# Wuziyi616/SlotDiffusion

Measured on AMD Instinct MI355X. Metric: train-step images/sec, 128x128 7-slot (DPM-Solver denoise-steps/sec in `denoise`), higher is better.
Workload: dtype bf16; 1 GPU; BASELINE configs[1]: img_based SlotDiffusion, CLEVRTex 128x128, 7 slots: train step = slot encoder + frozen VQ-VAE encode + q-sample + UNet eps + MSE, backward, clip, Adam (dropout 0.1); batch_per_gpu=64, hip_graph=True, parallelism=dp1

## Files before the change

include/sdmi.h:

```cpp
#ifndef SDMI_H_
#define SDMI_H_

#ifdef __cplusplus
extern "C" {
#endif

#define SDMI_VERSION 100

enum { SDMI_F32 = 0, SDMI_BF16 = 1, SDMI_FP8 = 2  };
enum { SDMI_ACT_NONE = 0, SDMI_ACT_RELU = 1, SDMI_ACT_SILU = 2, SDMI_ACT_GELU = 3 };
enum { SDMI_OK = 0, SDMI_EINVAL = -1, SDMI_ELAUNCH = -2, SDMI_EUNSUPPORTED = -3 };

int sdmi_version(void);
const char* sdmi_last_error(void);

typedef struct {
  const void* a;
  const void* w;
  void* out;
  const float* bias;
  const float* rowvec;
  const void* residual;
  float* workspace;
  int dtype, out_dtype;
// ... 21 lines not shown
  void* out2;
  int ldc2;
  int defer_epilogue;
  float* gn_part;
  int gn_groups;
  const float* alpha_dev;
  int parity4;
} SdmiGemmArgs;
int sdmi_igemm(const SdmiGemmArgs* a, void* stream);
int sdmi_igemm_split_plan(const SdmiGemmArgs* a, void* stream);
int sdmi_splitk_finish(const SdmiGemmArgs* a, void* stream);
enum {
  SDMI_ROUTE_NONE = 0,
  SDMI_ROUTE_CFG = 1,
  SDMI_ROUTE_DMA = 2,
  SDMI_ROUTE_SYM = 3,
  SDMI_ROUTE_HALO = 4,
  SDMI_ROUTE_C64 = 5
};
int sdmi_igemm_last_route(void);

typedef struct {
  const void* a;
  const void* dy;
  float* dw;
  float* dbias;
  float* workspace;
  int dtype;
  int M, N, K, lda, ldy;
  int B, H, W, Cin, Ho, Wo, KH, KW, stride, pad_t, pad_l, ups;
  int splits;
  int accumulate;
  int defer_fold;
} SdmiWgradArgs;
int sdmi_wgrad(const SdmiWgradArgs* a, void* stream);
enum {
  SDMI_WGRAD_KERNEL_IGEMM = 0,
  SDMI_WGRAD_KERNEL_C64 = 1,
  SDMI_WGRAD_KERNEL_HALO = 2,
  SDMI_WGRAD_KERNEL_F32_T128 = 3,
  SDMI_WGRAD_KERNEL_F32_T64 = 4
};
int sdmi_wgrad_kernel(const SdmiWgradArgs* a, void* stream);

typedef struct { const void* problems; int n; } SdmiWgradGroupArgs;
int sdmi_wgrad_group(const SdmiWgradGroupArgs* a, void* stream);
int sdmi_wgrad_fold_group(const SdmiWgradGroupArgs* a, void* stream);

typedef struct {
  const void* dgrad; const void* wgrad; const void* fold;
  int dgrad_cap, wgrad_tile;
} SdmiBwdPairArgs;
int sdmi_bwd_pair(const SdmiBwdPairArgs* a, void* stream);

typedef struct {
  const void* x;
  void* y;
  const float* gamma;
  const float* beta;
  float* stats;
  float* partial;
  int dtype;
  int B, HW, C, groups;
  float eps;
  int act;
  int nsplit;
  const void* residual;
  float drop_p;
  long long drop_seed;
  const long long* drop_seed_dev;
  void* y8;
  float y8_scale;
  const void* x2;
  int C1;
  const float* part;
  int part_splits;
  float part_alpha;
  const float* part_bias;
  const float* part_rowvec;
  int part_ldrv;
  const void* part_residual;
  void* raw_out;
} SdmiGroupNormArgs;
int sdmi_groupnorm_stats(const SdmiGroupNormArgs* a, void* stream);
int sdmi_groupnorm_apply(const SdmiGroupNormArgs* a, void* stream);
int sdmi_groupnorm(const SdmiGroupNormArgs* a, void* stream);

typedef struct {
  const void* x;
  const void* dy;
  void* dx;
  const float* gamma;
  const float* beta;
  const float* stats;
  float* dgamma;
  float* dbeta;
  float* partial;
  int dtype;
  int B, HW, C, groups;
  int act;
  int nsplit;
  const void* residual;
  void* dresidual;
  int accumulate;
  const void* dextra0;
  const void* dextra1;
  float drop_p;
  long long drop_seed;
  const long long* drop_seed_dev;
  float* dxsum;
  int ld_dxsum;
  int defer_colsum;
} SdmiGroupNormBwdArgs;
int sdmi_groupnorm_bwd(const SdmiGroupNormBwdArgs* a, void* stream);
int sdmi_groupnorm_bwd_fused(const SdmiGroupNormBwdArgs* a, void* unused);
int sdmi_groupnorm_bwd_entries(const SdmiGroupNormBwdArgs* a, void* stream);

typedef struct {
  const void* x; void* y; const float* gamma; const float* beta;
  float* stats;
  int dtype; int rows, C, ldx, ldy; float eps;
} SdmiLayerNormArgs;
int sdmi_layernorm(const SdmiLayerNormArgs* a, void* stream);

typedef struct {
  const void* x; const void* dy; void* dx; const float* gamma; const float* stats;
  float* dgamma; float* dbeta;
  float* partial;
  int dtype; int rows, C; int nblk; int accumulate;
  const void* dextra;
  int defer_colsum;
} SdmiLayerNormBwdArgs;
int sdmi_layernorm_bwd(const SdmiLayerNormBwdArgs* a, void* stream);

typedef struct { const float* partial; float* out0; float* out1; int nblk, C; } SdmiColsumItem;
typedef struct { const void* items; int n; } SdmiColsumGroupArgs;
int sdmi_colsum_group(const SdmiColsumGroupArgs* a, void* stream);


typedef struct {
  const void* q; const void* k; const void* v; void* out; float* lse;
  int dtype; int B, heads, Sq, Skv; int ldq, ldk, ldv, ldo; float scale;
  int head_dim;
} SdmiAttnArgs;
int sdmi_attention(const SdmiAttnArgs* a, void* stream);

typedef struct {
  const void* q; const void* k; const void* v; const void* out; const void* dout; const float* lse;
  void* dq; void* dk; void* dv;
  int dtype; int B, heads, Sq, Skv; int ldq, ldk, ldv, ldo; float scale;
  int head_dim;
} SdmiAttnBwdArgs;
int sdmi_attention_bwd(const SdmiAttnBwdArgs* a, void* stream);

typedef struct { void* x; int dtype; int rows, cols, ld; float scale; } SdmiSoftmaxArgs;
int sdmi_softmax_rows(const SdmiSoftmaxArgs* a, void* stream);

typedef struct {
  const void* k; const void* v;
  const float* slots_in;
  float* slots_out;
  float* seg;
  const float *lnq_g, *lnq_b, *wq;
  const float *w_ih, *w_hh, *b_ih, *b_hh;
  const float *lnm_g, *lnm_b, *w1, *b1, *w2, *b2;
  float* trace;
  int dtype; int B, M, N, D, Hid, iters, ldkv; long long slots_bstride; float eps, scale;
} SdmiSlotAttnArgs;
int sdmi_slot_attention(const SdmiSlotAttnArgs* a, void* stream);

typedef struct {
  const float* z; const float* codebook; long long* idx; float* zq;
  int R, dim, ldz, n_codes; float scale;
  const float* z2; float zc0, zc1, zdiv;
} SdmiVqArgs;
int sdmi_vq_nearest(const SdmiVqArgs* a, void* stream);

enum { SDMI_DPM_EPS = 0, SDMI_DPM_X0 = 1, SDMI_DPM_V = 2 };
enum { SDMI_DPM_UPD_NONE = 0, SDMI_DPM_UPD_FIRST = 1, SDMI_DPM_UPD_SINGLE = 2, SDMI_DPM_UPD_MULTI2 = 3,
       SDMI_DPM_UPD_MULTI3 = 4 };
typedef struct {
  const float* x; const float* out; const float* codebook;
  long long* idx; float* m0;
  const float* base; const float* h1; const float* h2; float* y;
  int R, n_codes, target, mode;
  float scale, sigma, alpha;
  float c0, c1, c2, c3, k0, k1, g, k2;
} SdmiDpmStepArgs;
int sdmi_dpm_step(const SdmiDpmStepArgs* a, void* stream);

typedef struct {
  const float* x; const float* out; const float* codebook;
  long long* idx; float* m0;
  int R, n_codes, target;
  float scale, sigma, alpha;
  const float* base; const float* h1; const float* h2; const float* h3;
  float* xc; float* y;
  int corr_order, pred_order;
  float c0, c1, w1, w2, wn;
  float p0, p1, q1, q2;
} SdmiUnipcStepArgs;
int sdmi_unipc_step(const SdmiUnipcStepArgs* a, void* stream);

enum { SDMI_X0_NONE = 0, SDMI_X0_CLAMP = 1, SDMI_X0_DYNAMIC = 2 };
enum { SDMI_PX_MAX_ROWS = 16384 };
typedef struct {
  const float* x; const float* out; float* m0;
  const float* base; const float* h1; const float* h2; float* y;
  int R, rows_per_sample, target, mode, correct, q_k;
  float q_w, max_val, sigma, alpha;
  float c0, c1, c2, c3, k0, k1, g, k2;
} SdmiDpmStepPxArgs;
int sdmi_dpm_step_px(const SdmiDpmStepPxArgs* a, void* stream);

typedef struct {
  const float* x; const float* out; float* m0;
  int R, rows_per_sample, target, correct, q_k;
  float q_w, max_val, sigma, alpha;
  const float* base; const float* h1; const float* h2; const float* h3;
  float* xc; float* y;
  int corr_order, pred_order;
  float c0, c1, w1, w2, wn;
  float p0, p1, q1, q2;
} SdmiUnipcStepPxArgs;
int sdmi_unipc_step_px(const SdmiUnipcStepPxArgs* a, void* stream);

typedef struct {
  float* y; const float* x0; const float* x1; const float* x2; const float* x3;
  float c0, c1, c2, div; long long n;
} SdmiLincombArgs;
int sdmi_lincomb(const SdmiLincombArgs* a, void* stream);
typedef struct {
  float* y; const float* x0; const float* x1; const float* ca; const float* cb; int B; long long per;
} SdmiRowLincombArgs;
int sdmi_row_lincomb(const SdmiRowLincombArgs* a, void* stream);

typedef struct { const float* src; void* dst; int dtype; int B, C, H, W, Cpad; } SdmiNchwToNhwcArgs;
int sdmi_nchw_to_nhwc(const SdmiNchwToNhwcArgs* a, void* stream);
typedef struct { const void* src; float* dst; int dtype; int B, C, H, W, Cpad; } SdmiNhwcToNchwArgs;
int sdmi_nhwc_to_nchw(const SdmiNhwcToNchwArgs* a, void* stream);
typedef struct {
  const void* src; void* dst; int src_dtype, dst_dtype; long long rows; int cols, lds, ldd;
  int zpad;
} SdmiCast2dArgs;
int sdmi_cast2d(const SdmiCast2dArgs* a, void* stream);
typedef struct {
  const void* src; void* dst; int src_dtype; long long rows; int cols, lds, ldd; float scale;
} SdmiQuantFp8Args;
int sdmi_quant_fp8(const SdmiQuantFp8Args* a, void* stream);
typedef struct { const void* src; void* dst; long long n; int block_begin; int pad_; } SdmiFp8Desc;
typedef struct {
  const void* descs; int n_desc; int src_dtype; int total_blocks;
  unsigned* amax_bits;
  float* inv_scale;
} SdmiFp8GroupArgs;
int sdmi_fp8_quant_group(const SdmiFp8GroupArgs* a, void* stream);
typedef struct {
  const void* x; void* tok; void* qkv; void* out;
  const float* gn_gamma; const float* gn_beta;
  const void* wstream_a; const float* vec_a;
  const void* wstream_b; const float* vec_b;
  const void* wstream_img; const float* vec_img;
  int B, S, C, slots, phase;
  float gn_eps, ln_eps, attn_scale;
  int rows;
  float* part; int ff_split;
} SdmiStBlockArgs;
int sdmi_st_block(const SdmiStBlockArgs* a, void* stream);

typedef struct {
  const void* x; void* qkv; void* out;
  const void* wstream_a; const float* vec_a;
  const void* wstream_b; const float* vec_b;
  int B, L, Lp, C, heads, ffn_dim, phase;
  float ln_eps, attn_scale;
} SdmiRolloutLayerArgs;
int sdmi_rollout_layer(const SdmiRolloutLayerArgs* a, void* stream);

enum { SDMI_AGG_SUM = 0, SDMI_AGG_MEAN = 1, SDMI_AGG_MAX = 2 };
typedef struct {
  const void* slots; const void* w1p; const float* b1; const float* w2; const float* b2;
  const float* label;
  float* frame_logits; float* logits; int* t_star; float* loss; float* dlogit;
  int B, T, N, C, F, agg, x_dtype, op_dtype, phase;
  float loss_weight;
} SdmiReadoutFwdArgs;
int sdmi_readout_fwd(const SdmiReadoutFwdArgs* a, void* stream);
typedef struct {
  const void* slots; const void* w1p; const float* b1; const float* w2;
  const int* t_star; const float* dlogit; const float* gscale;
  float* dw1; float* db1; float* dw2; float* db2;
  int B, T, N, C, F, agg, x_dtype, op_dtype, accumulate;
} SdmiReadoutBwdArgs;
int sdmi_readout_bwd(const SdmiReadoutBwdArgs* a, void* stream);

typedef struct {
  const void* x; void* out;
  void* hgn; float* gn_stats;
  void* tok; void* n1; float* st1; void* qkv;
  void* a1; float* lse1;
  void* x1; void* n2; float* st2;
  void* q2; void* a2; float* lse2;
  void* x2; void* n3; float* st3;
  void* h; void* g; void* x3;
  const void* kv2; int ldkv;
  const void* wstream_a; const void* wstream_b;
// ... 223 lines not shown
```

slotdiffusion_amd/csrc/attention_bwd.hip:

```cpp
#include "common.h"

namespace {

template <typename T, int HD>
__device__ __forceinline__ void load_row32(const T* p, float* f) {
  constexpr int VEC = Elem<T>::VEC;
#pragma unroll
  for (int c = 0; c < HD; c += VEC) unpack16<T>(*reinterpret_cast<const uint4*>(p + c), f + c);
}
template <typename T, int HD>
__device__ __forceinline__ void store_row32(T* p, const float* f) {
  constexpr int VEC = Elem<T>::VEC;
#pragma unroll
  for (int c = 0; c < HD; c += VEC) *reinterpret_cast<uint4*>(p + c) = pack16<T>(f + c);
}

template <typename T, int HD>
__global__ __launch_bounds__(256) void attn_bwd_dq_kernel(SdmiAttnBwdArgs p) {
  constexpr int VEC = Elem<T>::VEC;
  extern __shared__ __attribute__((aligned(16))) char smem[];
  float* Ks = reinterpret_cast<float*>(smem);
  float* Vs = Ks + p.Skv * HD;
  const int b = blockIdx.z, h = blockIdx.y, tid = threadIdx.x;
  {
    const int vpr = HD / VEC, total = p.Skv * vpr;
    const T* kb = (const T*)p.k + (long long)b * p.Skv * p.ldk + h * HD;
    const T* vb = (const T*)p.v + (long long)b * p.Skv * p.ldv + h * HD;
    for (int i = tid; i < total; i += blockDim.x) {
      const int row = i / vpr, c = (i % vpr) * VEC;
      float f[VEC];
      unpack16<T>(*reinterpret_cast<const uint4*>(kb + (long long)row * p.ldk + c), f);
#pragma unroll
      for (int j = 0; j < VEC; ++j) Ks[row * HD + c + j] = f[j];
      unpack16<T>(*reinterpret_cast<const uint4*>(vb + (long long)row * p.ldv + c), f);
#pragma unroll
      for (int j = 0; j < VEC; ++j) Vs[row * HD + c + j] = f[j];
    }
  }
  __syncthreads();
  const int qi = blockIdx.x * blockDim.x + tid;
  if (qi >= p.Sq) return;
  float q[HD], dO[HD], o[HD], dq[HD];
  load_row32<T, HD>((const T*)p.q + ((long long)b * p.Sq + qi) * p.ldq + h * HD, q);
  load_row32<T, HD>((const T*)p.dout + ((long long)b * p.Sq + qi) * p.ldo + h * HD, dO);
  load_row32<T, HD>((const T*)p.out + ((long long)b * p.Sq + qi) * p.ldo + h * HD, o);
  float D = 0.f;
#pragma unroll
  for (int d = 0; d < HD; ++d) { D += dO[d] * o[d]; dq[d] = 0.f; q[d] *= p.scale; }
  const float lse = p.lse[((long long)b * p.heads + h) * p.Sq + qi];
  for (int j = 0; j < p.Skv; ++j) {
    float s = 0.f, dp = 0.f;
#pragma unroll
    for (int d = 0; d < HD; ++d) { s += q[d] * Ks[j * HD + d]; dp += dO[d] * Vs[j * HD + d]; }
    const float ds = __expf(s - lse) * (dp - D);
#pragma unroll
    for (int d = 0; d < HD; ++d) dq[d] += ds * Ks[j * HD + d];
  }
#pragma unroll
  for (int d = 0; d < HD; ++d) dq[d] *= p.scale;
  store_row32<T, HD>((T*)p.dq + ((long long)b * p.Sq + qi) * p.ldq + h * HD, dq);
}

template <typename T, int HD>
__global__ __launch_bounds__(256) void attn_bwd_dkv_kernel(SdmiAttnBwdArgs p) {
  constexpr int VEC = Elem<T>::VEC;
  constexpr int QC = 64;
  __shared__ float Qs[QC][HD], Os[QC][HD], Ts[QC][HD], Ls[QC], Ds[QC];
  const int b = blockIdx.z, h = blockIdx.y, tid = threadIdx.x;
  const int kj = blockIdx.x * blockDim.x + tid;
  const bool act = kj < p.Skv;
  float k[HD], v[HD], dk[HD], dv[HD];
  if (act) {
    load_row32<T, HD>((const T*)p.k + ((long long)b * p.Skv + kj) * p.ldk + h * HD, k);
    load_row32<T, HD>((const T*)p.v + ((long long)b * p.Skv + kj) * p.ldv + h * HD, v);
  }
#pragma unroll
  for (int d = 0; d < HD; ++d) { dk[d] = dv[d] = 0.f; if (!act) k[d] = v[d] = 0.f; }
  for (int q0 = 0; q0 < p.Sq; q0 += QC) {
    __syncthreads();
    const int vpr = HD / VEC;
    for (int i = tid; i < QC * vpr; i += blockDim.x) {
      const int r = i / vpr, c = (i % vpr) * VEC, qi = q0 + r;
      float fq[VEC], fo[VEC], fout[VEC];
      if (qi < p.Sq) {
        const long long ro = ((long long)b * p.Sq + qi);
        unpack16<T>(*reinterpret_cast<const uint4*>((const T*)p.q + ro * p.ldq + h * HD + c), fq);
        unpack16<T>(*reinterpret_cast<const uint4*>((const T*)p.dout + ro * p.ldo + h * HD + c), fo);
        unpack16<T>(*reinterpret_cast<const uint4*>((const T*)p.out + ro * p.ldo + h * HD + c), fout);
      } else {
#pragma unroll
        for (int j = 0; j < VEC; ++j) fq[j] = fo[j] = fout[j] = 0.f;
      }
#pragma unroll
      for (int j = 0; j < VEC; ++j) { Qs[r][c + j] = fq[j]; Os[r][c + j] = fo[j]; Ts[r][c + j] = fout[j]; }
    }
    __syncthreads();
    for (int r = tid; r < QC; r += blockDim.x) {
      const int qi = q0 + r;
      float D = 0.f;
#pragma unroll
      for (int d = 0; d < HD; ++d) D += Os[r][d] * Ts[r][d];
      Ds[r] = D;
      Ls[r] = qi < p.Sq ? p.lse[((long long)b * p.heads + h) * p.Sq + qi] : INFINITY;
    }
    __syncthreads();
    const int qn = min(QC, p.Sq - q0);
    for (int r = 0; r < qn; ++r) {
      float s = 0.f, dp = 0.f;
#pragma unroll
      for (int d = 0; d < HD; ++d) { s += Qs[r][d] * k[d]; dp += Os[r][d] * v[d]; }
      const float pij = __expf(s * p.scale - Ls[r]);
      const float ds = pij * (dp - Ds[r]);
#pragma unroll
      for (int d = 0; d < HD; ++d) { dv[d] += pij * Os[r][d]; dk[d] += ds * Qs[r][d]; }
    }
  }
  if (!act) return;
#pragma unroll
  for (int d = 0; d < HD; ++d) dk[d] *= p.scale;
  store_row32<T, HD>((T*)p.dk + ((long long)b * p.Skv + kj) * p.ldk + h * HD, dk);
  store_row32<T, HD>((T*)p.dv + ((long long)b * p.Skv + kj) * p.ldv + h * HD, dv);
}

template <typename T, int HD>
__global__ __launch_bounds__(512) void attn_bwd_dkv_small_kernel(SdmiAttnBwdArgs p) {
  const int b = blockIdx.y, h = blockIdx.x;
  const int j = threadIdx.x / HD, d = threadIdx.x % HD;
  const float kd = Elem<T>::ld((const T*)p.k + ((long long)b * p.Skv + j) * p.ldk + h * HD + d);
  const float vd = Elem<T>::ld((const T*)p.v + ((long long)b * p.Skv + j) * p.ldv + h * HD + d);
  const float* lse = p.lse + ((long long)b * p.heads + h) * p.Sq;
  float dk = 0.f, dv = 0.f;
  for (int i = 0; i < p.Sq; ++i) {
    const long long ro = (long long)b * p.Sq + i;
    const float qd = Elem<T>::ld((const T*)p.q + ro * p.ldq + h * HD + d);
    const float od = Elem<T>::ld((const T*)p.dout + ro * p.ldo + h * HD + d);
    const float outd = Elem<T>::ld((const T*)p.out + ro * p.ldo + h * HD + d);
    float s = qd * kd, dp = od * vd, D = od * outd;
#pragma unroll
    for (int o = 16; o > 0; o >>= 1) {
      s += __shfl_xor(s, o, 64);
      dp += __shfl_xor(dp, o, 64);
      D += __shfl_xor(D, o, 64);
    }
    const float pij = __expf(s * p.scale - lse[i]);
    dv += pij * od;
    dk += pij * (dp - D) * qd;
  }
  Elem<T>::st((T*)p.dk + ((long long)b * p.Skv + j) * p.ldk + h * HD + d, dk * p.scale);
  Elem<T>::st((T*)p.dv + ((long long)b * p.Skv + j) * p.ldv + h * HD + d, dv);
}

template <typename T, int HD>
int launch_attn_bwd(const SdmiAttnBwdArgs& a, hipStream_t st) {
  int threads = ((a.Sq + 63) / 64) * 64;
  if (threads > 256) threads = 256;
  dim3 grid((a.Sq + threads - 1) / threads, a.heads, a.B);
  const int smem = 2 * a.Skv * HD * 4;
  SDMI_OPTIN_LDS((attn_bwd_dq_kernel<T, HD>), (2 * 512 * HD * 4 < 160 * 1024 ? 2 * 512 * HD * 4 : 160 * 1024),
                 "attention_bwd");
  hipLaunchKernelGGL((attn_bwd_dq_kernel<T, HD>), grid, dim3(threads), smem, st, a);
  if (a.Skv <= 16 && HD == 32) {
    hipLaunchKernelGGL((attn_bwd_dkv_small_kernel<T, HD>), dim3(a.heads, a.B), dim3(a.Skv * HD), 0,
                       st, a);
  } else {
    int kt = ((a.Skv + 63) / 64) * 64;
    if (kt > 256) kt = 256;
    dim3 g2((a.Skv + kt - 1) / kt, a.heads, a.B);
    hipLaunchKernelGGL((attn_bwd_dkv_kernel<T, HD>), g2, dim3(kt), 0, st, a);
  }
  return sdmi_check_launch("attention_bwd");
}


typedef short b_s16x4 __attribute__((ext_vector_type(4)));
typedef short b_s16x8 __attribute__((ext_vector_type(8)));
#define ATB_LDS_V4(p) ((__attribute__((address_space(3))) b_s16x4*)(p))
constexpr int P80 = 80, P64 = 64;

__device__ __forceinline__ unsigned bpack2(float lo, float hi) {
  return (unsigned)f32_to_bf16(lo) | ((unsigned)f32_to_bf16(hi) << 16);
}
__device__ __forceinline__ bf16x8 bpack8(const float* v) {
  const u32x4 w = {bpack2(v[0], v[1]), bpack2(v[2], v[3]), bpack2(v[4], v[5]), bpack2(v[6], v[7])};
  return __builtin_bit_cast(bf16x8, w);
}
__device__ __forceinline__ bf16x8 tr_operand(const char* img_lane, int row0) {
  const char* q = img_lane + row0 * P64;
  const b_s16x4 lo = __builtin_amdgcn_ds_read_tr16_b64_v4i16(ATB_LDS_V4(q));
  const b_s16x4 hi = __builtin_amdgcn_ds_read_tr16_b64_v4i16(ATB_LDS_V4(q + 8 * P64));
  const b_s16x8 v = __builtin_shufflevector(lo, hi, 0, 1, 2, 3, 4, 5, 6, 7);
  return __builtin_bit_cast(bf16x8, v);
}
__device__ __forceinline__ float dot8(const u32x4& a, const u32x4& b) {
  float fa[8], fb[8];
  unpack16<bf16_t>(reinterpret_cast<const uint4&>(a), fa);
  unpack16<bf16_t>(reinterpret_cast<const uint4&>(b), fb);
  float s = 0.f;
#pragma unroll
  for (int i = 0; i < 8; ++i) s += fa[i] * fb[i];
  return s;
}
__device__ __forceinline__ void store_col(bf16_t* rp, const f32x16& acc, float sc) {
#pragma unroll
  for (int j = 0; j < 4; ++j) {
    uint2 w;
    w.x = bpack2(acc[4 * j] * sc, acc[4 * j + 1] * sc);
    w.y = bpack2(acc[4 * j + 2] * sc, acc[4 * j + 3] * sc);
    *reinterpret_cast<uint2*>(rp + 8 * j) = w;
  }
}

constexpr int ATB_CHUNK = 512;

__device__ __forceinline__ void attn_bwd_dq_mfma_body(const SdmiAttnBwdArgs& p, char* smem, int bx, int chunk) {
  const int skv_pad = (p.Skv + 31) / 32 * 32;
  const int cap = skv_pad < chunk ? skv_pad : chunk;
  char* K80 = smem;
  char* K64 = K80 + cap * P80;
  char* V80 = K64 + cap * P64;
  const int b = blockIdx.z, h = blockIdx.y;
  const int tid = threadIdx.x, lane = tid & 63, wave = tid >> 6;
  const int q0 = (bx * 4 + wave) * 32;
  const bool active = q0 < p.Sq;
  const int ql = lane & 31, hh = lane >> 5;
  const int qi = q0 + ql, qc = qi < p.Sq ? qi : p.Sq - 1;
  bf16x8 bq[2], bdo[2];
  float D;
  {
    const long long ro = (long long)b * p.Sq + qc;
    const bf16_t* qp = (const bf16_t*)p.q + ro * p.ldq + h * 32 + hh * 8;
    const bf16_t* dp_ = (const bf16_t*)p.dout + ro * p.ldo + h * 32 + hh * 8;
    const bf16_t* op = (const bf16_t*)p.out + ro * p.ldo + h * 32 + hh * 8;
    const u32x4 q0v = *reinterpret_cast<const u32x4*>(qp), q1v = *reinterpret_cast<const u32x4*>(qp + 16);
    const u32x4 d0v = *reinterpret_cast<const u32x4*>(dp_), d1v = *reinterpret_cast<const u32x4*>(dp_ + 16);
    const u32x4 o0v = *reinterpret_cast<const u32x4*>(op), o1v = *reinterpret_cast<const u32x4*>(op + 16);
    bq[0] = __builtin_bit_cast(bf16x8, q0v); bq[1] = __builtin_bit_cast(bf16x8, q1v);
    bdo[0] = __builtin_bit_cast(bf16x8, d0v); bdo[1] = __builtin_bit_cast(bf16x8, d1v);
    D = dot8(d0v, o0v) + dot8(d1v, o1v);
    D += __shfl_xor(D, 32, 64);
  }
  const float lse = p.lse[((long long)b * p.heads + h) * p.Sq + qc];
  f32x16 dq;
#pragma unroll
  for (int r = 0; r < 16; ++r) dq[r] = 0.f;
  const int g = lane >> 4, t = lane & 15;
  const char* kfrag = K80 + ql * P80 + hh * 16;
  const char* vfrag = V80 + ql * P80 + hh * 16;
  const char* ktr = K64 + (4 * hh + (t >> 2)) * P64 + ((g & 1) * 16 + (t & 3) * 4) * 2;
  const bf16_t* kbase = (const bf16_t*)p.k + (long long)b * p.Skv * p.ldk + h * 32;
  const bf16_t* vbase = (const bf16_t*)p.v + (long long)b * p.Skv * p.ldv + h * 32;
  for (int c0 = 0; c0 < skv_pad; c0 += chunk) {
    const int rows = skv_pad - c0 < chunk ? skv_pad - c0 : chunk;
    if (c0) __syncthreads();
    {
      const u32x4 zero4 = {0u, 0u, 0u, 0u};
      for (int i = tid; i < rows * 4; i += 256) {
        const int row = i >> 2, c = i & 3;
        const bool ok = c0 + row < p.Skv;
        const u32x4 kv = ok ? *reinterpret_cast<const u32x4*>(kbase + (long long)(c0 + row) * p.ldk + c * 8) : zero4;
        const u32x4 vv = ok ? *reinterpret_cast<const u32x4*>(vbase + (long long)(c0 + row) * p.ldv + c * 8) : zero4;
        *reinterpret_cast<u32x4*>(K80 + row * P80 + c * 16) = kv;
        *reinterpret_cast<u32x4*>(K64 + row * P64 + c * 16) = kv;
        *reinterpret_cast<u32x4*>(V80 + row * P80 + c * 16) = vv;
      }
    }
    __syncthreads();
    if (!active) continue;
    for (int kb = 0; kb < rows / 32; ++kb) {
      f32x16 s, dp;
#pragma unroll
      for (int r = 0; r < 16; ++r) s[r] = dp[r] = 0.f;
#pragma unroll
      for (int ks = 0; ks < 2; ++ks) {
        const u32x4 ak = *reinterpret_cast<const u32x4*>(kfrag + kb * 32 * P80 + ks * 32);
        const u32x4 av = *reinterpret_cast<const u32x4*>(vfrag + kb * 32 * P80 + ks * 32);
        s = __builtin_amdgcn_mfma_f32_32x32x16_bf16(__builtin_bit_cast(bf16x8, ak), bq[ks], s, 0, 0, 0);
        dp = __builtin_amdgcn_mfma_f32_32x32x16_bf16(__builtin_bit_cast(bf16x8, av), bdo[ks], dp, 0, 0, 0);
      }
      float ds[16];
#pragma unroll
      for (int r = 0; r < 16; ++r) {
        const int key = c0 + kb * 32 + (r & 3) + 8 * (r >> 2) + 4 * hh;
        const float pr = key < p.Skv ? __expf(s[r] * p.scale - lse) : 0.f;
        ds[r] = pr * (dp[r] - D);
      }
#pragma unroll
      for (int mm = 0; mm < 2; ++mm)
        dq = __builtin_amdgcn_mfma_f32_32x32x16_bf16(tr_operand(ktr, kb * 32 + 16 * mm),
                                                     bpack8(ds + 8 * mm), dq, 0, 0, 0);
    }
  }
  if (active && qi < p.Sq)
    store_col((bf16_t*)p.dq + ((long long)b * p.Sq + qi) * p.ldq + h * 32 + 4 * hh, dq, p.scale);
}

__device__ __forceinline__ void attn_bwd_dkv_mfma_body(const SdmiAttnBwdArgs& p, char* smem, int bx, int chunk) {
  const int sq_pad = (p.Sq + 31) / 32 * 32;
  const int cap = sq_pad < chunk ? sq_pad : chunk;
  char* Q80 = smem;
  char* Q64 = Q80 + cap * P80;
  char* O80 = Q64 + cap * P64;
  char* O64 = O80 + cap * P80;
  float* lse_s = reinterpret_cast<float*>(O64 + cap * P64);
  float* D_s = lse_s + cap;
  const int b = blockIdx.z, h = blockIdx.y;
  const int tid = threadIdx.x, lane = tid & 63, wave = tid >> 6;
  const int k0 = (bx * 4 + wave) * 32;
  const bool active = k0 < p.Skv;
  const int kl = lane & 31, hh = lane >> 5;
  const int kj = k0 + kl, kc = kj < p.Skv ? kj : p.Skv - 1;
  bf16x8 bk[2], bv[2];
  {
    const bf16_t* kp = (const bf16_t*)p.k + ((long long)b * p.Skv + kc) * p.ldk + h * 32 + hh * 8;
    const bf16_t* vp = (const bf16_t*)p.v + ((long long)b * p.Skv + kc) * p.ldv + h * 32 + hh * 8;
    bk[0] = __builtin_bit_cast(bf16x8, *reinterpret_cast<const u32x4*>(kp));
    bk[1] = __builtin_bit_cast(bf16x8, *reinterpret_cast<const u32x4*>(kp + 16));
    bv[0] = __builtin_bit_cast(bf16x8, *reinterpret_cast<const u32x4*>(vp));
    bv[1] = __builtin_bit_cast(bf16x8, *reinterpret_cast<const u32x4*>(vp + 16));
  }
  f32x16 dk, dv;
#pragma unroll
  for (int r = 0; r < 16; ++r) dk[r] = dv[r] = 0.f;
  const int g = lane >> 4, t = lane & 15;
  const char* qfrag = Q80 + kl * P80 + hh * 16;
  const char* ofrag = O80 + kl * P80 + hh * 16;
  const int troff = (4 * hh + (t >> 2)) * P64 + ((g & 1) * 16 + (t & 3) * 4) * 2;
  const char* qtr = Q64 + troff;
  const char* otr = O64 + troff;
  const bf16_t* qb_ = (const bf16_t*)p.q + (long long)b * p.Sq * p.ldq + h * 32;
  const bf16_t* db = (const bf16_t*)p.dout + (long long)b * p.Sq * p.ldo + h * 32;
  const bf16_t* ob = (const bf16_t*)p.out + (long long)b * p.Sq * p.ldo + h * 32;
  for (int c0 = 0; c0 < sq_pad; c0 += chunk) {
    const int rows = sq_pad - c0 < chunk ? sq_pad - c0 : chunk;
    if (c0) __syncthreads();
    {
      const u32x4 zero4 = {0u, 0u, 0u, 0u};
      for (int i = tid; i < rows * 4; i += 256) {
        const int row = i >> 2, c = i & 3;
        const bool ok = c0 + row < p.Sq;
        const u32x4 qv = ok ? *reinterpret_cast<const u32x4*>(qb_ + (long long)(c0 + row) * p.ldq + c * 8) : zero4;
        const u32x4 dv4 = ok ? *reinterpret_cast<const u32x4*>(db + (long long)(c0 + row) * p.ldo + c * 8) : zero4;
        *reinterpret_cast<u32x4*>(Q80 + row * P80 + c * 16) = qv;
        *reinterpret_cast<u32x4*>(Q64 + row * P64 + c * 16) = qv;
        *reinterpret_cast<u32x4*>(O80 + row * P80 + c * 16) = dv4;
        *reinterpret_cast<u32x4*>(O64 + row * P64 + c * 16) = dv4;
      }
      for (int r = tid; r < rows; r += 256) {
        const int qi = c0 + r;
        float d = 0.f, l = INFINITY;
        if (qi < p.Sq) {
#pragma unroll
          for (int c = 0; c < 4; ++c)
            d += dot8(*reinterpret_cast<const u32x4*>(db + (long long)qi * p.ldo + c * 8),
                      *reinterpret_cast<const u32x4*>(ob + (long long)qi * p.ldo + c * 8));
          l = p.lse[((long long)b * p.heads + h) * p.Sq + qi];
        }
        D_s[r] = d;
        lse_s[r] = l;
      }
    }
    __syncthreads();
    if (!active) continue;
    for (int qb = 0; qb < rows / 32; ++qb) {
      f32x16 s, dp;
#pragma unroll
      for (int r = 0; r < 16; ++r) s[r] = dp[r] = 0.f;
#pragma unroll
      for (int ks = 0; ks < 2; ++ks) {
        const u32x4 aq = *reinterpret_cast<const u32x4*>(qfrag + qb * 32 * P80 + ks * 32);
        const u32x4 ao = *reinterpret_cast<const u32x4*>(ofrag + qb * 32 * P80 + ks * 32);
        s = __builtin_amdgcn_mfma_f32_32x32x16_bf16(__builtin_bit_cast(bf16x8, aq), bk[ks], s, 0, 0, 0);
        dp = __builtin_amdgcn_mfma_f32_32x32x16_bf16(__builtin_bit_cast(bf16x8, ao), bv[ks], dp, 0, 0, 0);
      }
      float pr[16], ds[16];
#pragma unroll
      for (int j = 0; j < 4; ++j) {
        const f32x4 l4 = *reinterpret_cast<const f32x4*>(lse_s + qb * 32 + 8 * j + 4 * hh);
        const f32x4 d4 = *reinterpret_cast<const f32x4*>(D_s + qb * 32 + 8 * j + 4 * hh);
#pragma unroll
        for (int i = 0; i < 4; ++i) {
          const int r = 4 * j + i;
          pr[r] = __expf(s[r] * p.scale - l4[i]);
          ds[r] = pr[r] * (dp[r] - d4[i]);
        }
      }
#pragma unroll
      for (int mm = 0; mm < 2; ++mm) {
        dv = __builtin_amdgcn_mfma_f32_32x32x16_bf16(tr_operand(otr, qb * 32 + 16 * mm),
                                                     bpack8(pr + 8 * mm), dv, 0, 0, 0);
        dk = __builtin_amdgcn_mfma_f32_32x32x16_bf16(tr_operand(qtr, qb * 32 + 16 * mm),
                                                     bpack8(ds + 8 * mm), dk, 0, 0, 0);
      }
    }
  }
  if (active && kj < p.Skv) {
    store_col((bf16_t*)p.dk + ((long long)b * p.Skv + kj) * p.ldk + h * 32 + 4 * hh, dk, p.scale);
    store_col((bf16_t*)p.dv + ((long long)b * p.Skv + kj) * p.ldv + h * 32 + 4 * hh, dv, 1.f);
  }
}

__global__ __launch_bounds__(256) void attn_bwd_mfma_kernel(SdmiAttnBwdArgs p, int nqx, int chunk_k, int chunk_q) {
  extern __shared__ __attribute__((aligned(16))) char smem[];
  if ((int)blockIdx.x < nqx) attn_bwd_dq_mfma_body(p, smem, blockIdx.x, chunk_k);
  else attn_bwd_dkv_mfma_body(p, smem, (int)blockIdx.x - nqx, chunk_q);
}

int launch_attn_bwd_mfma(const SdmiAttnBwdArgs& a, hipStream_t st) {
  SDMI_OPTIN_LDS(attn_bwd_mfma_kernel, 160 * 1024, "attention_bwd (mfma)");
  int skv_pad = (a.Skv + 31) / 32 * 32, sq_pad = (a.Sq + 31) / 32 * 32;
  if (skv_pad > ATB_CHUNK) skv_pad = ATB_CHUNK;
  const int qmax = a.Skv <= 32 ? 128 : ATB_CHUNK;
  if (sq_pad > qmax) sq_pad = qmax;
  const int smem_q = skv_pad * (2 * P80 + P64), smem_k = sq_pad * (2 * P80 + 2 * P64 + 8);
  const int nqx = (a.Sq + 127) / 128, nkx = (a.Skv + 127) / 128;
  hipLaunchKernelGGL(attn_bwd_mfma_kernel, dim3(nqx + nkx, a.heads, a.B), dim3(256),
                     smem_q > smem_k ? smem_q : smem_k, st, a, nqx, skv_pad, sq_pad);
  return sdmi_check_launch("attention_bwd (mfma)");
}

}

extern "C" int sdmi_attention_bwd(const SdmiAttnBwdArgs* a, void* stream) {
  SDMI_REQUIRE(a && a->q && a->k && a->v && a->out && a->dout && a->lse && a->dq && a->dk && a->dv,
               "null pointer");
  const int vec = a->dtype == SDMI_BF16 ? 8 : 4;
  SDMI_REQUIRE(a->ldq % vec == 0 && a->ldk % vec == 0 && a->ldv % vec == 0 && a->ldo % vec == 0,
               "row pitches must keep 16-byte alignment");
  const int hd = a->head_dim > 0 ? a->head_dim : 32;
  SDMI_REQUIRE(hd == 32 || hd == 48, "head_dim must be 32 or 48");
  hipStream_t st = (hipStream_t)stream;
  if (a->dtype == SDMI_BF16 && hd == 32) {
    SDMI_REQUIRE(a->Skv >= 1, "Skv must be positive");
    return launch_attn_bwd_mfma(*a, st);
  }
  SDMI_REQUIRE(a->Skv >= 1 && a->Skv <= 400, "Skv must be in [1, 400] (fp32 / head_dim 48: K/V staged whole in LDS)");
  if (a->dtype == SDMI_BF16)
    return hd == 32 ? launch_attn_bwd<bf16_t, 32>(*a, st) : launch_attn_bwd<bf16_t, 48>(*a, st);
  return hd == 32 ? launch_attn_bwd<float, 32>(*a, st) : launch_attn_bwd<float, 48>(*a, st);
}
```

Baseline: 2375 images/s.

## Add single-block-per-head fused MFMA attention backward for short sequences

Adds a new attention-backward kernel that handles one (batch, head) per workgroup when Sq and Skv are at most 256. It stages K/V and Q/dO once in LDS, and each wave does either a dQ row tile or a dK/dV column tile, so the old chunked loop with separate dq and dkv block groups is avoided. It also pairs heads to remap block indices, skips key masking on full tiles, and uses a paired bf16 pack intrinsic. The new path is on by default and can be turned off with an env var. The cost is large blocks (up to 1024 threads) with heavy LDS use per block, which may reduce occupancy.

```diff
diff --git a/include/sdmi.h b/include/sdmi.h
--- a/include/sdmi.h
+++ b/include/sdmi.h
@@ -197,6 +197,12 @@
   int head_dim;
 } SdmiAttnBwdArgs;
 int sdmi_attention_bwd(const SdmiAttnBwdArgs* a, void* stream);
+enum {
+  SDMI_ATTN_BWD_KERNEL_VALU = 0,
+  SDMI_ATTN_BWD_KERNEL_MFMA = 1,
+  SDMI_ATTN_BWD_KERNEL_HEAD = 2
+};
+int sdmi_attention_bwd_kernel(const SdmiAttnBwdArgs* a, void* stream);
 
 typedef struct { void* x; int dtype; int rows, cols, ld; float scale; } SdmiSoftmaxArgs;
 int sdmi_softmax_rows(const SdmiSoftmaxArgs* a, void* stream);
diff --git a/slotdiffusion_amd/csrc/attention_bwd.hip b/slotdiffusion_amd/csrc/attention_bwd.hip
--- a/slotdiffusion_amd/csrc/attention_bwd.hip
+++ b/slotdiffusion_amd/csrc/attention_bwd.hip
@@ -1,3 +1,4 @@
+#include <stdlib.h>
 #include "common.h"
 
 namespace {
@@ -178,7 +179,7 @@
 constexpr int P80 = 80, P64 = 64;
 
 __device__ __forceinline__ unsigned bpack2(float lo, float hi) {
-  return (unsigned)f32_to_bf16(lo) | ((unsigned)f32_to_bf16(hi) << 16);
+  return f32x2_to_bf16x2(lo, hi);
 }
 __device__ __forceinline__ bf16x8 bpack8(const float* v) {
   const u32x4 w = {bpack2(v[0], v[1]), bpack2(v[2], v[3]), bpack2(v[4], v[5]), bpack2(v[6], v[7])};
@@ -207,6 +208,146 @@
     w.x = bpack2(acc[4 * j] * sc, acc[4 * j + 1] * sc);
     w.y = bpack2(acc[4 * j + 2] * sc, acc[4 * j + 3] * sc);
     *reinterpret_cast<uint2*>(rp + 8 * j) = w;
+  }
+}
+
+
+__device__ __forceinline__ void load_frag2(const bf16_t* rp, u32x4& lo, u32x4& hi) {
+  lo = *reinterpret_cast<const u32x4*>(rp);
+  hi = *reinterpret_cast<const u32x4*>(rp + 16);
+}
+
+__device__ __forceinline__ void dq_wave_rows(const SdmiAttnBwdArgs& p, int b, int h, int qc, int hh,
+                                             bf16x8* bq, bf16x8* bdo, float& D, float& lse) {
+  const long long ro = (long long)b * p.Sq + qc;
+  u32x4 q0v, q1v, d0v, d1v, o0v, o1v;
+  load_frag2((const bf16_t*)p.q + ro * p.ldq + h * 32 + hh * 8, q0v, q1v);
+  load_frag2((const bf16_t*)p.dout + ro * p.ldo + h * 32 + hh * 8, d0v, d1v);
+  load_frag2((const bf16_t*)p.out + ro * p.ldo + h * 32 + hh * 8, o0v, o1v);
+  bq[0] = __builtin_bit_cast(bf16x8, q0v); bq[1] = __builtin_bit_cast(bf16x8, q1v);
+  bdo[0] = __builtin_bit_cast(bf16x8, d0v); bdo[1] = __builtin_bit_cast(bf16x8, d1v);
+  D = dot8(d0v, o0v) + dot8(d1v, o1v);
+  D += __shfl_xor(D, 32, 64);
+  lse = p.lse[((long long)b * p.heads + h) * p.Sq + qc];
+}
+
+__device__ __forceinline__ void stage_kv(const SdmiAttnBwdArgs& p, const bf16_t* kbase, const bf16_t* vbase,
+                                         char* K80, char* K64, char* V80, int c0, int rows, int tid, int nthr) {
+  const u32x4 zero4 = {0u, 0u, 0u, 0u};
+  for (int i = tid; i < rows * 4; i += nthr) {
+    const int row = i >> 2, c = i & 3;
+    const bool ok = c0 + row < p.Skv;
+    const u32x4 kv = ok ? *reinterpret_cast<const u32x4*>(kbase + (long long)(c0 + row) * p.ldk + c * 8) : zero4;
+    const u32x4 vv = ok ? *reinterpret_cast<const u32x4*>(vbase + (long long)(c0 + row) * p.ldv + c * 8) : zero4;
+    *reinterpret_cast<u32x4*>(K80 + row * P80 + c * 16) = kv;
+    *reinterpret_cast<u32x4*>(K64 + row * P64 + c * 16) = kv;
+    *reinterpret_cast<u32x4*>(V80 + row * P80 + c * 16) = vv;
+  }
+}
+
+__device__ __forceinline__ void dq_wave_block(const SdmiAttnBwdArgs& p, const char* kfrag, const char* vfrag,
+                                              const char* ktr, int kb, int key0, int hh, const bf16x8* bq,
+                                              const bf16x8* bdo, float D, float lse, f32x16& dq) {
+  f32x16 s, dp;
+#pragma unroll
+  for (int r = 0; r < 16; ++r) s[r] = dp[r] = 0.f;
+#pragma unroll
+  for (int ks = 0; ks < 2; ++ks) {
+    const u32x4 ak = *reinterpret_cast<const u32x4*>(kfrag + kb * 32 * P80 + ks * 32);
+    const u32x4 av = *reinterpret_cast<const u32x4*>(vfrag + kb * 32 * P80 + ks * 32);
+    s = __builtin_amdgcn_mfma_f32_32x32x16_bf16(__builtin_bit_cast(bf16x8, ak), bq[ks], s, 0, 0, 0);
+    dp = __builtin_amdgcn_mfma_f32_32x32x16_bf16(__builtin_bit_cast(bf16x8, av), bdo[ks], dp, 0, 0, 0);
+  }
+  float ds[16];
+  if (key0 + 32 <= p.Skv) {
+#pragma unroll
+    for (int r = 0; r < 16; ++r) ds[r] = __expf(s[r] * p.scale - lse) * (dp[r] - D);
+  } else {
+#pragma unroll
+    for (int r = 0; r < 16; ++r) {
+      const int key = key0 + (r & 3) + 8 * (r >> 2) + 4 * hh;
+      const float pr = key < p.Skv ? __expf(s[r] * p.scale - lse) : 0.f;
+      ds[r] = pr * (dp[r] - D);
+    }
+  }
+#pragma unroll
+  for (int mm = 0; mm < 2; ++mm)
+    dq = __builtin_amdgcn_mfma_f32_32x32x16_bf16(tr_operand(ktr, kb * 32 + 16 * mm),
+                                                 bpack8(ds + 8 * mm), dq, 0, 0, 0);
+}
+
+__device__ __forceinline__ void dkv_wave_rows(const SdmiAttnBwdArgs& p, int b, int h, int kc, int hh,
+                                              bf16x8* bk, bf16x8* bv) {
+  u32x4 k0v, k1v, v0v, v1v;
+  load_frag2((const bf16_t*)p.k + ((long long)b * p.Skv + kc) * p.ldk + h * 32 + hh * 8, k0v, k1v);
+  load_frag2((const bf16_t*)p.v + ((long long)b * p.Skv + kc) * p.ldv + h * 32 + hh * 8, v0v, v1v);
+  bk[0] = __builtin_bit_cast(bf16x8, k0v); bk[1] = __builtin_bit_cast(bf16x8, k1v);
+  bv[0] = __builtin_bit_cast(bf16x8, v0v); bv[1] = __builtin_bit_cast(bf16x8, v1v);
+}
+
+__device__ __forceinline__ void stage_qo(const SdmiAttnBwdArgs& p, const bf16_t* qb_, const bf16_t* db,
+                                         const bf16_t* ob, const float* lse_g, char* Q80, char* Q64, char* O80,
+                                         char* O64, float* lse_s, float* D_s, int c0, int rows, int tid, int nthr) {
+  const u32x4 zero4 = {0u, 0u, 0u, 0u};
+  for (int i = tid; i < rows * 4; i += nthr) {
+    const int row = i >> 2, c = i & 3;
+    const bool ok = c0 + row < p.Sq;
+    const u32x4 qv = ok ? *reinterpret_cast<const u32x4*>(qb_ + (long long)(c0 + row) * p.ldq + c * 8) : zero4;
+    const u32x4 dv4 = ok ? *reinterpret_cast<const u32x4*>(db + (long long)(c0 + row) * p.ldo + c * 8) : zero4;
+    *reinterpret_cast<u32x4*>(Q80 + row * P80 + c * 16) = qv;
+    *reinterpret_cast<u32x4*>(Q64 + row * P64 + c * 16) = qv;
+    *reinterpret_cast<u32x4*>(O80 + row * P80 + c * 16) = dv4;
+    *reinterpret_cast<u32x4*>(O64 + row * P64 + c * 16) = dv4;
+  }
+  for (int r = tid; r < rows; r += nthr) {
+    const int qi = c0 + r;
+    float d = 0.f, l = INFINITY;
+    if (qi < p.Sq) {
+#pragma unroll
+      for (int c = 0; c < 4; ++c)
+        d += dot8(*reinterpret_cast<const u32x4*>(db + (long long)qi * p.ldo + c * 8),
+                  *reinterpret_cast<const u32x4*>(ob + (long long)qi * p.ldo + c * 8));
+      l = lse_g[qi];
+    }
+    D_s[r] = d;
+    lse_s[r] = l;
+  }
+}
+
+template <bool TIGHT = false>
+__device__ __forceinline__ void dkv_wave_block(const SdmiAttnBwdArgs& p, const char* qfrag, const char* ofrag,
+                                               const char* qtr, const char* otr, const float* lse_s,
+                                               const float* D_s, int qb, int hh, const bf16x8* bk,
+                                               const bf16x8* bv, f32x16& dk, f32x16& dv) {
+  f32x16 s, dp;
+#pragma unroll
+  for (int r = 0; r < 16; ++r) s[r] = dp[r] = 0.f;
+#pragma unroll
+  for (int ks = 0; ks < 2; ++ks) {
+    const u32x4 aq = *reinterpret_cast<const u32x4*>(qfrag + qb * 32 * P80 + ks * 32);
+    const u32x4 ao = *reinterpret_cast<const u32x4*>(ofrag + qb * 32 * P80 + ks * 32);
+    s = __builtin_amdgcn_mfma_f32_32x32x16_bf16(__builtin_bit_cast(bf16x8, aq), bk[ks], s, 0, 0, 0);
+    dp = __builtin_amdgcn_mfma_f32_32x32x16_bf16(__builtin_bit_cast(bf16x8, ao), bv[ks], dp, 0, 0, 0);
+  }
+  float pr[16], ds[16];
+#pragma unroll
+  for (int j = 0; j < 4; ++j) {
+    const f32x4 l4 = *reinterpret_cast<const f32x4*>(lse_s + qb * 32 + 8 * j + 4 * hh);
+    const f32x4 d4 = *reinterpret_cast<const f32x4*>(D_s + qb * 32 + 8 * j + 4 * hh);
+#pragma unroll
+    for (int i = 0; i < 4; ++i) {
+      const int r = 4 * j + i;
+      pr[r] = __expf(s[r] * p.scale - l4[i]);
+      ds[r] = pr[r] * (dp[r] - d4[i]);
+    }
+    if (TIGHT && j == 1) __builtin_amdgcn_sched_barrier(0);
+  }
+#pragma unroll
+  for (int mm = 0; mm < 2; ++mm) {
+    dv = __builtin_amdgcn_mfma_f32_32x32x16_bf16(tr_operand(otr, qb * 32 + 16 * mm),
+                                                 bpack8(pr + 8 * mm), dv, 0, 0, 0);
+    dk = __builtin_amdgcn_mfma_f32_32x32x16_bf16(tr_operand(qtr, qb * 32 + 16 * mm),
+                                                 bpack8(ds + 8 * mm), dk, 0, 0, 0);
   }
 }
 
@@ -225,21 +366,8 @@
   const int ql = lane & 31, hh = lane >> 5;
   const int qi = q0 + ql, qc = qi < p.Sq ? qi : p.Sq - 1;
   bf16x8 bq[2], bdo[2];
-  float D;
-  {
-    const long long ro = (long long)b * p.Sq + qc;
-    const bf16_t* qp = (const bf16_t*)p.q + ro * p.ldq + h * 32 + hh * 8;
-    const bf16_t* dp_ = (const bf16_t*)p.dout + ro * p.ldo + h * 32 + hh * 8;
-    const bf16_t* op = (const bf16_t*)p.out + ro * p.ldo + h * 32 + hh * 8;
-    const u32x4 q0v = *reinterpret_cast<const u32x4*>(qp), q1v = *reinterpret_cast<const u32x4*>(qp + 16);
-    const u32x4 d0v = *reinterpret_cast<const u32x4*>(dp_), d1v = *reinterpret_cast<const u32x4*>(dp_ + 16);
-    const u32x4 o0v = *reinterpret_cast<const u32x4*>(op), o1v = *reinterpret_cast<const u32x4*>(op + 16);
-    bq[0] = __builtin_bit_cast(bf16x8, q0v); bq[1] = __builtin_bit_cast(bf16x8, q1v);
-    bdo[0] = __builtin_bit_cast(bf16x8, d0v); bdo[1] = __builtin_bit_cast(bf16x8, d1v);
-    D = dot8(d0v, o0v) + dot8(d1v, o1v);
-    D += __shfl_xor(D, 32, 64);
-  }
-  const float lse = p.lse[((long long)b * p.heads + h) * p.Sq + qc];
+  float D, lse;
+  dq_wave_rows(p, b, h, qc, hh, bq, bdo, D, lse);
   f32x16 dq;
 #pragma unroll
   for (int r = 0; r < 16; ++r) dq[r] = 0.f;
@@ -252,43 +380,11 @@
   for (int c0 = 0; c0 < skv_pad; c0 += chunk) {
     const int rows = skv_pad - c0 < chunk ? skv_pad - c0 : chunk;
     if (c0) __syncthreads();
-    {
-      const u32x4 zero4 = {0u, 0u, 0u, 0u};
-      for (int i = tid; i < rows * 4; i += 256) {
-        const int row = i >> 2, c = i & 3;
-        const bool ok = c0 + row < p.Skv;
-        const u32x4 kv = ok ? *reinterpret_cast<const u32x4*>(kbase + (long long)(c0 + row) * p.ldk + c * 8) : zero4;
-        const u32x4 vv = ok ? *reinterpret_cast<const u32x4*>(vbase + (long long)(c0 + row) * p.ldv + c * 8) : zero4;
-        *reinterpret_cast<u32x4*>(K80 + row * P80 + c * 16) = kv;
-        *reinterpret_cast<u32x4*>(K64 + row * P64 + c * 16) = kv;
-        *reinterpret_cast<u32x4*>(V80 + row * P80 + c * 16) = vv;
-      }
-    }
+    stage_kv(p, kbase, vbase, K80, K64, V80, c0, rows, tid, 256);
     __syncthreads();
     if (!active) continue;
-    for (int kb = 0; kb < rows / 32; ++kb) {
-      f32x16 s, dp;
-#pragma unroll
-      for (int r = 0; r < 16; ++r) s[r] = dp[r] = 0.f;
-#pragma unroll
-      for (int ks = 0; ks < 2; ++ks) {
-        const u32x4 ak = *reinterpret_cast<const u32x4*>(kfrag + kb * 32 * P80 + ks * 32);
-        const u32x4 av = *reinterpret_cast<const u32x4*>(vfrag + kb * 32 * P80 + ks * 32);
-        s = __builtin_amdgcn_mfma_f32_32x32x16_bf16(__builtin_bit_cast(bf16x8, ak), bq[ks], s, 0, 0, 0);
-        dp = __builtin_amdgcn_mfma_f32_32x32x16_bf16(__builtin_bit_cast(bf16x8, av), bdo[ks], dp, 0, 0, 0);
-      }
-      float ds[16];
-#pragma unroll
-      for (int r = 0; r < 16; ++r) {
-        const int key = c0 + kb * 32 + (r & 3) + 8 * (r >> 2) + 4 * hh;
-        const float pr = key < p.Skv ? __expf(s[r] * p.scale - lse) : 0.f;
-        ds[r] = pr * (dp[r] - D);
-      }
-#pragma unroll
-      for (int mm = 0; mm < 2; ++mm)
-        dq = __builtin_amdgcn_mfma_f32_32x32x16_bf16(tr_operand(ktr, kb * 32 + 16 * mm),
-                                                     bpack8(ds + 8 * mm), dq, 0, 0, 0);
-    }
+    for (int kb = 0; kb < rows / 32; ++kb)
+      dq_wave_block(p, kfrag, vfrag, ktr, kb, c0 + kb * 32, hh, bq, bdo, D, lse, dq);
   }
   if (active && qi < p.Sq)
     store_col((bf16_t*)p.dq + ((long long)b * p.Sq + qi) * p.ldq + h * 32 + 4 * hh, dq, p.scale);
@@ -310,14 +406,7 @@
   const int kl = lane & 31, hh = lane >> 5;
   const int kj = k0 + kl, kc = kj < p.Skv ? kj : p.Skv - 1;
   bf16x8 bk[2], bv[2];
-  {
-    const bf16_t* kp = (const bf16_t*)p.k + ((long long)b * p.Skv + kc) * p.ldk + h * 32 + hh * 8;
-    const bf16_t* vp = (const bf16_t*)p.v + ((long long)b * p.Skv + kc) * p.ldv + h * 32 + hh * 8;
-    bk[0] = __builtin_bit_cast(bf16x8, *reinterpret_cast<const u32x4*>(kp));
-    bk[1] = __builtin_bit_cast(bf16x8, *reinterpret_cast<const u32x4*>(kp + 16));
-    bv[0] = __builtin_bit_cast(bf16x8, *reinterpret_cast<const u32x4*>(vp));
-    bv[1] = __builtin_bit_cast(bf16x8, *reinterpret_cast<const u32x4*>(vp + 16));
-  }
+  dkv_wave_rows(p, b, h, kc, hh, bk, bv);
   f32x16 dk, dv;
 #pragma unroll
   for (int r = 0; r < 16; ++r) dk[r] = dv[r] = 0.f;
@@ -330,68 +419,15 @@
   const bf16_t* qb_ = (const bf16_t*)p.q + (long long)b * p.Sq * p.ldq + h * 32;
   const bf16_t* db = (const bf16_t*)p.dout + (long long)b * p.Sq * p.ldo + h * 32;
   const bf16_t* ob = (const bf16_t*)p.out + (long long)b * p.Sq * p.ldo + h * 32;
+  const float* lse_g = p.lse + ((long long)b * p.heads + h) * p.Sq;
   for (int c0 = 0; c0 < sq_pad; c0 += chunk) {
     const int rows = sq_pad - c0 < chunk ? sq_pad - c0 : chunk;
     if (c0) __syncthreads();
-    {
-      const u32x4 zero4 = {0u, 0u, 0u, 0u};
-      for (int i = tid; i < rows * 4; i += 256) {
-        const int row = i >> 2, c = i & 3;
-        const bool ok = c0 + row < p.Sq;
-        const u32x4 qv = ok ? *reinterpret_cast<const u32x4*>(qb_ + (long long)(c0 + row) * p.ldq + c * 8) : zero4;
-        const u32x4 dv4 = ok ? *reinterpret_cast<const u32x4*>(db + (long long)(c0 + row) * p.ldo + c * 8) : zero4;
-        *reinterpret_cast<u32x4*>(Q80 + row * P80 + c * 16) = qv;
-        *reinterpret_cast<u32x4*>(Q64 + row * P64 + c * 16) = qv;
-        *reinterpret_cast<u32x4*>(O80 + row * P80 + c * 16) = dv4;
-        *reinterpret_cast<u32x4*>(O64 + row * P64 + c * 16) = dv4;
-      }
-      for (int r = tid; r < rows; r += 256) {
-        const int qi = c0 + r;
-        float d = 0.f, l = INFINITY;
-        if (qi < p.Sq) {
-#pragma unroll
-          for (int c = 0; c < 4; ++c)
-            d += dot8(*reinterpret_cast<const u32x4*>(db + (long long)qi * p.ldo + c * 8),
-                      *reinterpret_cast<const u32x4*>(ob + (long long)qi * p.ldo + c * 8));
-          l = p.lse[((long long)b * p.heads + h) * p.Sq + qi];
-        }
-        D_s[r] = d;
-        lse_s[r] = l;
-      }
-    }
+    stage_qo(p, qb_, db, ob, lse_g, Q80, Q64, O80, O64, lse_s, D_s, c0, rows, tid, 256);
     __syncthreads();
     if (!active) continue;
-    for (int qb = 0; qb < rows / 32; ++qb) {
-      f32x16 s, dp;
-#pragma unroll
-      for (int r = 0; r < 16; ++r) s[r] = dp[r] = 0.f;
-#pragma unroll
-      for (int ks = 0; ks < 2; ++ks) {
-        const u32x4 aq = *reinterpret_cast<const u32x4*>(qfrag + qb * 32 * P80 + ks * 32);
-        const u32x4 ao = *reinterpret_cast<const u32x4*>(ofrag + qb * 32 * P80 + ks * 32);
-        s = __builtin_amdgcn_mfma_f32_32x32x16_bf16(__builtin_bit_cast(bf16x8, aq), bk[ks], s, 0, 0, 0);
-        dp = __builtin_amdgcn_mfma_f32_32x32x16_bf16(__builtin_bit_cast(bf16x8, ao), bv[ks], dp, 0, 0, 0);
-      }
-      float pr[16], ds[16];
-#pragma unroll
-      for (int j = 0; j < 4; ++j) {
-        const f32x4 l4 = *reinterpret_cast<const f32x4*>(lse_s + qb * 32 + 8 * j + 4 * hh);
-        const f32x4 d4 = *reinterpret_cast<const f32x4*>(D_s + qb * 32 + 8 * j + 4 * hh);
-#pragma unroll
-        for (int i = 0; i < 4; ++i) {
-          const int r = 4 * j + i;
-          pr[r] = __expf(s[r] * p.scale - l4[i]);
-          ds[r] = pr[r] * (dp[r] - d4[i]);
-        }
-      }
-#pragma unroll
-      for (int mm = 0; mm < 2; ++mm) {
-        dv = __builtin_amdgcn_mfma_f32_32x32x16_bf16(tr_operand(otr, qb * 32 + 16 * mm),
-                                                     bpack8(pr + 8 * mm), dv, 0, 0, 0);
-        dk = __builtin_amdgcn_mfma_f32_32x32x16_bf16(tr_operand(qtr, qb * 32 + 16 * mm),
-                                                     bpack8(ds + 8 * mm), dk, 0, 0, 0);
-      }
-    }
+    for (int qb = 0; qb < rows / 32; ++qb)
+      dkv_wave_block(p, qfrag, ofrag, qtr, otr, lse_s, D_s, qb, hh, bk, bv, dk, dv);
   }
   if (active && kj < p.Skv) {
     store_col((bf16_t*)p.dk + ((long long)b * p.Skv + kj) * p.ldk + h * 32 + 4 * hh, dk, p.scale);
@@ -418,23 +454,146 @@
   return sdmi_check_launch("attention_bwd (mfma)");
 }
 
+constexpr int ATH_MAX = 256;
+
+__device__ __forceinline__ int fresh_lane(int tid) {
+  asm volatile("" : "+v"(tid));
+  return tid & 63;
+}
+__device__ __forceinline__ int tr_lane_offset(int lane) {
+  const int hh = lane >> 5, g = lane >> 4, t = lane & 15;
+  return (4 * hh + (t >> 2)) * P64 + ((g & 1) * 16 + (t & 3) * 4) * 2;
+}
+
+template <int MAXT>
+__global__ __launch_bounds__(MAXT) void attn_bwd_head_kernel(SdmiAttnBwdArgs p, int pair_heads) {
+  extern __shared__ __attribute__((aligned(16))) char smem[];
+  const int skv_pad = (p.Skv + 31) / 32 * 32, sq_pad = (p.Sq + 31) / 32 * 32;
+  char* K80 = smem;
+  char* K64 = K80 + skv_pad * P80;
+  char* V80 = K64 + skv_pad * P64;
+  char* Q80 = V80 + skv_pad * P80;
+  char* Q64 = Q80 + sq_pad * P80;
+  char* O80 = Q64 + sq_pad * P64;
+  char* O64 = O80 + sq_pad * P80;
+  float* lse_s = reinterpret_cast<float*>(O64 + sq_pad * P64);
+  float* D_s = lse_s + sq_pad;
+  int b = blockIdx.z, h = blockIdx.y;
+  if (pair_heads) {
+    const int l = blockIdx.y + p.heads * blockIdx.z, pp = (l >> 4) * 8 + (l & 7), hp = p.heads >> 1;
+    b = pp / hp;
+    h = 2 * (pp % hp) + ((l >> 3) & 1);
+  }
+  const int tid = threadIdx.x, nthr = blockDim.x;
+  const int wave = __builtin_amdgcn_readfirstlane(tid >> 6), nq = sq_pad / 32;
+  const bool is_dq = wave < nq;
+  const int r0 = (is_dq ? wave : wave - nq) * 32;
+  bf16x8 fa[2], fb[2];
+  float D = 0.f, lse = 0.f;
+  {
+    const int ri = r0 + (tid & 31), hh = (tid >> 5) & 1;
+    if (is_dq) dq_wave_rows(p, b, h, ri < p.Sq ? ri : p.Sq - 1, hh, fa, fb, D, lse);
+    else dkv_wave_rows(p, b, h, ri < p.Skv ? ri : p.Skv - 1, hh, fa, fb);
+  }
+  stage_kv(p, (const bf16_t*)p.k + (long long)b * p.Skv * p.ldk + h * 32,
+           (const bf16_t*)p.v + (long long)b * p.Skv * p.ldv + h * 32, K80, K64, V80, 0, skv_pad, tid, nthr);
+  stage_qo(p, (const bf16_t*)p.q + (long long)b * p.Sq * p.ldq + h * 32,
+           (const bf16_t*)p.dout + (long long)b * p.Sq * p.ldo + h * 32,
+           (const bf16_t*)p.out + (long long)b * p.Sq * p.ldo + h * 32, p.lse + ((long long)b * p.heads + h) * p.Sq,
+           Q80, Q64, O80, O64, lse_s, D_s, 0, sq_pad, tid, nthr);
+  __syncthreads();
+  if (is_dq) {
+    f32x16 dq;
+#pragma unroll
+    for (int r = 0; r < 16; ++r) dq[r] = 0.f;
+    {
+      const int lane = fresh_lane(tid), rl = lane & 31, hh = lane >> 5;
+      const char* kfrag = K80 + rl * P80 + hh * 16;
+      const char* vfrag = V80 + rl * P80 + hh * 16;
+      const char* ktr = K64 + tr_lane_offset(lane);
+      for (int kb = 0; kb < skv_pad / 32; ++kb)
+        dq_wave_block(p, kfrag, vfrag, ktr, kb, kb * 32, hh, fa, fb, D, lse, dq);
+    }
+    const int lane = fresh_lane(tid), qi = r0 + (lane & 31), hh = lane >> 5;
+    if (qi < p.Sq)
+      store_col((bf16_t*)p.dq + ((long long)b * p.Sq + qi) * p.ldq + h * 32 + 4 * hh, dq, p.scale);
+  } else {
+    f32x16 dk, dv;
+#pragma unroll
+    for (int r = 0; r < 16; ++r) dk[r] = dv[r] = 0.f;
+    {
+      const int lane = fresh_lane(tid), rl = lane & 31, hh = lane >> 5;
+      const char* qfrag = Q80 + rl * P80 + hh * 16;
+      const char* ofrag = O80 + rl * P80 + hh * 16;
+      const char* qtr = Q64 + tr_lane_offset(lane);
+      const char* otr = O64 + tr_lane_offset(lane);
+      for (int qb = 0; qb < sq_pad / 32; ++qb)
+        dkv_wave_block<(MAXT > 512)>(p, qfrag, ofrag, qtr, otr, lse_s, D_s, qb, hh, fa, fb, dk, dv);
+    }
+    const int lane = fresh_lane(tid), kj = r0 + (lane & 31), hh = lane >> 5;
+    if (kj < p.Skv) {
+      store_col((bf16_t*)p.dk + ((long long)b * p.Skv + kj) * p.ldk + h * 32 + 4 * hh, dk, p.scale);
+      store_col((bf16_t*)p.dv + ((long long)b * p.Skv + kj) * p.ldv + h * 32 + 4 * hh, dv, 1.f);
+    }
+  }
+}
+
+int launch_attn_bwd_head(const SdmiAttnBwdArgs& a, hipStream_t st) {
+  const int skv_pad = (a.Skv + 31) / 32 * 32, sq_pad = (a.Sq + 31) / 32 * 32;
+  const int smem = skv_pad * (2 * P80 + P64) + sq_pad * (2 * P80 + 2 * P64 + 8);
+  const int threads = (sq_pad / 32 + skv_pad / 32) * 64;
+  const dim3 grid(1, a.heads, a.B);
+  const int pair_heads = a.heads % 2 == 0 && (a.heads * a.B) % 16 == 0;
+  if (threads <= 512) {
+    SDMI_OPTIN_LDS(attn_bwd_head_kernel<512>, 160 * 1024, "attention_bwd (head)");
+    hipLaunchKernelGGL(attn_bwd_head_kernel<512>, grid, dim3(threads), smem, st, a, pair_heads);
+  } else {
+    SDMI_OPTIN_LDS(attn_bwd_head_kernel<1024>, 160 * 1024, "attention_bwd (head)");
+    hipLaunchKernelGGL(attn_bwd_head_kernel<1024>, grid, dim3(threads), smem, st, a, pair_heads);
+  }
+  return sdmi_check_launch("attention_bwd (head)");
+}
+
+int select_attn_bwd(const SdmiAttnBwdArgs& a) {
+  const int hd = a.head_dim > 0 ? a.head_dim : 32;
+  if (a.dtype != SDMI_BF16 || hd != 32) return SDMI_ATTN_BWD_KERNEL_VALU;
+  const char* e = getenv("SDMI_ATTN_BWD_HEAD");
+  const bool head = e ? atoi(e) != 0 : true;
+  if (head && a.Sq >= 1 && a.Sq <= ATH_MAX && a.Skv <= ATH_MAX) return SDMI_ATTN_BWD_KERNEL_HEAD;
+  return SDMI_ATTN_BWD_KERNEL_MFMA;
+}
+
+const char* attn_bwd_geometry_error(const SdmiAttnBwdArgs& a) {
+  const int vec = a.dtype == SDMI_BF16 ? 8 : 4;
+  if (a.ldq % vec != 0 || a.ldk % vec != 0 || a.ldv % vec != 0 || a.ldo % vec != 0)
+    return "row pitches must keep 16-byte alignment";
+  const int hd = a.head_dim > 0 ? a.head_dim : 32;
+  if (hd != 32 && hd != 48) return "head_dim must be 32 or 48";
+  if (a.dtype == SDMI_BF16 && hd == 32) return a.Skv >= 1 ? nullptr : "Skv must be positive";
+  if (a.Skv < 1 || a.Skv > 400) return "Skv must be in [1, 400] (fp32 / head_dim 48: K/V staged whole in LDS)";
+  return nullptr;
+}
+
 }
 
 extern "C" int sdmi_attention_bwd(const SdmiAttnBwdArgs* a, void* stream) {
   SDMI_REQUIRE(a && a->q && a->k && a->v && a->out && a->dout && a->lse && a->dq && a->dk && a->dv,
                "null pointer");
-  const int vec = a->dtype == SDMI_BF16 ? 8 : 4;
-  SDMI_REQUIRE(a->ldq % vec == 0 && a->ldk % vec == 0 && a->ldv % vec == 0 && a->ldo % vec == 0,
-               "row pitches must keep 16-byte alignment");
+  const char* err = attn_bwd_geometry_error(*a);
+  SDMI_REQUIRE(!err, err);
   const int hd = a->head_dim > 0 ? a->head_dim : 32;
-  SDMI_REQUIRE(hd == 32 || hd == 48, "head_dim must be 32 or 48");
   hipStream_t st = (hipStream_t)stream;
-  if (a->dtype == SDMI_BF16 && hd == 32) {
-    SDMI_REQUIRE(a->Skv >= 1, "Skv must be positive");
-    return launch_attn_bwd_mfma(*a, st);
-  }
-  SDMI_REQUIRE(a->Skv >= 1 && a->Skv <= 400, "Skv must be in [1, 400] (fp32 / head_dim 48: K/V staged whole in LDS)");
+  const int which = select_attn_bwd(*a);
+  if (which == SDMI_ATTN_BWD_KERNEL_HEAD) return launch_attn_bwd_head(*a, st);
+  if (which == SDMI_ATTN_BWD_KERNEL_MFMA) return launch_attn_bwd_mfma(*a, st);
   if (a->dtype == SDMI_BF16)
     return hd == 32 ? launch_attn_bwd<bf16_t, 32>(*a, st) : launch_attn_bwd<bf16_t, 48>(*a, st);
   return hd == 32 ? launch_attn_bwd<float, 32>(*a, st) : launch_attn_bwd<float, 48>(*a, st);
 }
+
+extern "C" int sdmi_attention_bwd_kernel(const SdmiAttnBwdArgs* a, void*) {
+  SDMI_REQUIRE(a, "null pointer");
+  const char* err = attn_bwd_geometry_error(*a);
+  SDMI_REQUIRE(!err, err);
+  return select_attn_bwd(*a);
+}
```

New measurement: 2390 images/s (median of 4 runs). About the same (+0.6%).
